# 3dhumangan/3DHumanGAN

Measured on NVIDIA H100. Metric: images_per_sec_G_fwd_512x512, higher is better.
Workload: dtype f32 (bf16x3 split on wgmma, fp32 accumulate)

## Files before the change

3dhumangan_b200/csrc/synth.cu:

```cuda
#include "common.cuh"
#include "wgmma.cuh"

namespace hg {

constexpr int kC = 256;
constexpr int kSynThreads = 384;
constexpr int kSynStages = 2;
constexpr int kASlots = 2;
constexpr int kXSlots = 5;
constexpr int kXs = 3;
constexpr int kSs = 2;
constexpr uint32_t kAChunk = 128 * 128;
constexpr uint32_t kBStage = 256 * 128;
constexpr uint32_t kXSlice = 32 * 128 * 4;

struct SpadeArgs {
  const float* x;
  long x_bstride;
  const float* mod;
  const float* scsh;
  const float* p_lr;
  long p_stride;
  const float* p_bias;
  const uint8_t* wgb;
  const float* bgb;
  const uint8_t* wimg;
  const float* bias;
  const float* skip;
  long skip_bstride;
  float* out;
  double* stats;
  const float* rgb_w;
  const float* rgb_b;
  const float* rgb_in;
  float* rgb_out;
  int B, HW, Hg, Wg, Rh, Rw;
  int nkc;
  int xC;
  const float* x2;
  float slope;
  int cout;
  int out_pm;
  int act;
  const float* ascale;
  const float* rk_v;
  int rk_n;
  const float* mod2;
};

struct SynSmem {
  uint8_t* a_hi;
  uint8_t* a_lo;
  uint8_t* b_st;
  float* x_st;
  int xs_n, ss_n;
  float* tab_g1;
  float* tab_g0;
  float* tab_bias;
  float* tab_rgbw;
  float* tab_bgb;
  float* tab_as;
  float* st_sum;
  float* st_sq;
  uint64_t* bars;
};

template <bool kPixel>
__device__ __forceinline__ SynSmem carve(uint8_t* raw) {
  constexpr int kA = kPixel ? 3 : kASlots, kX = kPixel ? 3 : kXSlots;
  uint8_t* s = reinterpret_cast<uint8_t*>((reinterpret_cast<uintptr_t>(raw) + 1023) & ~uintptr_t(1023));
  SynSmem m;
  m.a_hi = s;
  m.a_lo = s + kA * kAChunk;
  m.b_st = s + 2 * kA * kAChunk;
  m.x_st = reinterpret_cast<float*>(m.b_st + kSynStages * kBStage);
  m.xs_n = kPixel ? 2 : kXs;
  m.ss_n = kPixel ? 1 : kSs;
  float* f = m.x_st + kX * (kXSlice / 4);
  m.tab_g1 = f; f += kC;
  m.tab_g0 = f; f += kC;
  m.tab_bias = f; f += kC;
  m.tab_rgbw = f; f += 3 * kC;
  m.tab_bgb = f; f += 512;
  m.tab_as = f; f += kC;
  m.st_sum = f; f += kC;
  m.st_sq = f; f += kC;
  m.bars = reinterpret_cast<uint64_t*>(f);
  return m;
}
constexpr uint32_t kSynSmemBytes = 2 * kASlots * kAChunk + kSynStages * kBStage + kXSlots * kXSlice +
                                   (kC * 9 + 512) * 4 + 24 * 8 + 1024;
constexpr uint32_t kPixSmemBytes = 2 * 3 * kAChunk + kSynStages * kBStage + 3 * kXSlice + (kC * 9 + 512) * 4 + 24 * 8 + 1024;
static_assert(kSynSmemBytes <= 232448 && kPixSmemBytes <= 232448, "shared memory budget");

enum { B_FULL = 0 , B_EMPTY = 2 , X_FULL = 4 , X_EMPTY = 12  };

__device__ __forceinline__ void rows_barrier() { named_barrier(1, 256); }

__device__ __forceinline__ float lrelu02(float v) { return v > 0.f ? v : 0.2f * v; }

__device__ __forceinline__ float reduce_2pi(float t) {
  const float y = t * 0.15915494309189535f;
  const float k = (y + 12582912.f) - 12582912.f;
  float r = fmaf(-k, 6.2831854820251465f, t);
  return fmaf(-k, -1.7484555314695172e-07f, r);
}
__device__ __forceinline__ float sin_red(float t) { return __sinf(reduce_2pi(t)); }
__device__ __forceinline__ float cos_red(float t) { return __cosf(reduce_2pi(t)); }
__device__ __forceinline__ float2 reduce_2pi2(float2 t) {
  const float2 y = fmul2(t, make_float2(0.15915494309189535f, 0.15915494309189535f));
  const float2 k = fadd2(fadd2(y, make_float2(12582912.f, 12582912.f)), make_float2(-12582912.f, -12582912.f));
  const float2 r = ffma2(k, make_float2(-6.2831854820251465f, -6.2831854820251465f), t);
  return ffma2(k, make_float2(1.7484555314695172e-07f, 1.7484555314695172e-07f), r);
}
__device__ __forceinline__ float2 sin_red2(float2 t) { const float2 r = reduce_2pi2(t); return make_float2(__sinf(r.x), __sinf(r.y)); }
__device__ __forceinline__ float2 cos_red2(float2 t) { const float2 r = reduce_2pi2(t); return make_float2(__cosf(r.x), __cosf(r.y)); }

struct TileMap {
  int T, first, stride, count;
  __device__ __forceinline__ void get(int it, int& b, int& ti) const {
    const int tile = first + it * stride;
    b = tile / T;
    ti = tile - b * T;
  }
};

__device__ __forceinline__ void init_common(const SpadeArgs& a, const SynSmem& m) {
  for (int i = threadIdx.x; i < kC; i += blockDim.x) {
    m.tab_bias[i] = a.bias[i];
    m.st_sum[i] = 0.f;
    m.st_sq[i] = 0.f;
  }
  if (a.rgb_w)
    for (int i = threadIdx.x; i < 3 * kC; i += blockDim.x) m.tab_rgbw[i] = a.rgb_w[i];
  if (threadIdx.x == 0) {
    for (int i = 0; i < kSynStages; ++i) {
      mbar_init(m.bars + B_FULL + i, 1);
      mbar_init(m.bars + B_EMPTY + i, 2);
    }
    for (int i = 0; i < m.xs_n + m.ss_n; ++i) {
      mbar_init(m.bars + X_FULL + i, 1);
      mbar_init(m.bars + X_EMPTY + i, 8);
    }
    fence_mbar_init();
  }
  __syncthreads();
}

template <int kPasses>
__device__ __forceinline__ void weight_producer_loop(const SynSmem& m, const uint8_t* img, int nstages, int num_my_tiles) {
  uint32_t st = 0, ph = 0;
  for (int t = 0; t < num_my_tiles; ++t)
    for (int s = 0; s < nstages; ++s) {
      if (kPasses == 1 && (s & 1)) continue;
      mbar_wait_backoff(m.bars + B_EMPTY + st, ph ^ 1);
      mbar_arrive_expect_tx(m.bars + B_FULL + st, kBStage);
      bulk_g2s(m.b_st + st * kBStage, img + static_cast<size_t>(s) * kBStage, kBStage, m.bars + B_FULL + st);
      if (++st == kSynStages) { st = 0; ph ^= 1; }
    }
}

struct Pipe {
  uint32_t st = 0, ph = 0, prev = ~0u;
};
template <int N, int kPasses>
__device__ __forceinline__ void pipe_chunk(const SynSmem& m, Pipe& p, float (&d)[N / 2], uint32_t a_hi, uint32_t a_lo, bool accumulate,
                                           int t) {
#pragma unroll
  for (int part = 0; part < (kPasses == 3 ? 2 : 1); ++part) {
    mbar_wait(m.bars + B_FULL + p.st, p.ph);
    acc_fence(d);
    wgmma_fence();
    const uint32_t bt = smem_u32(m.b_st + p.st * kBStage);
    if (part == 0) {
      wg_k64<N>(d, a_hi, bt, accumulate);
      if (kPasses == 3) wg_k64<N>(d, a_lo, bt, true);
    } else {
      wg_k64<N>(d, a_hi, bt, true);
    }
    wgmma_commit();
    wgmma_wait<1>();
    acc_fence(d);
    if (p.prev != ~0u && t == 0) mbar_arrive(m.bars + B_EMPTY + p.prev);
    p.prev = p.st;
    if (++p.st == kSynStages) { p.st = 0; p.ph ^= 1; }
  }
}
template <int N>
__device__ __forceinline__ void pipe_drain(const SynSmem& m, Pipe& p, float (&d)[N / 2], int t) {
  wgmma_wait<0>();
  acc_fence(d);
  if (p.prev != ~0u && t == 0) mbar_arrive(m.bars + B_EMPTY + p.prev);
  p.prev = ~0u;
}

__device__ __forceinline__ void ring_emit(const SynSmem& m, uint32_t& g, int base, int slots, const float* src) {
  const uint32_t slot = base + g % slots;
  mbar_wait_backoff(m.bars + X_EMPTY + slot, ((g / slots) & 1) ^ 1);
  mbar_arrive_expect_tx(m.bars + X_FULL + slot, kXSlice);
  bulk_g2s(m.x_st + slot * (kXSlice / 4), src, kXSlice, m.bars + X_FULL + slot);
  ++g;
}
__device__ __forceinline__ void x_producer_loop(const SpadeArgs& a, const SynSmem& m, const TileMap& tm) {
  uint32_t g = 0;
  for (int it = 0; it < tm.count; ++it) {
    int b, ti;
    tm.get(it, b, ti);
    const int per_src = a.xC / 32;
    const float* base = a.x + static_cast<long>(b) * a.x_bstride + static_cast<long>(ti) * a.xC * 128;
    const float* base2 = a.x2 ? a.x2 + (static_cast<long>(b) * tm.T + ti) * a.xC * 128 : nullptr;
    for (int j = 0; j < 2 * a.nkc; ++j)
      ring_emit(m, g, 0, m.xs_n, (j < per_src ? base : base2 - per_src * 32 * 128) + j * 32 * 128);
  }
}
__device__ __forceinline__ void skip_producer_loop(const SpadeArgs& a, const SynSmem& m, const TileMap& tm) {
  if (!a.skip) return;
  uint32_t g = 0;
  for (int it = 0; it < tm.count; ++it) {
    int b, ti;
    tm.get(it, b, ti);
    const float* base = a.skip + static_cast<long>(b) * a.skip_bstride + static_cast<long>(ti) * a.cout * 128;
    for (int j = 0; j < a.cout / 32; ++j) ring_emit(m, g, m.xs_n, m.ss_n, base + j * 32 * 128);
  }
}

__device__ __forceinline__ uint32_t ring_take(const SynSmem& m, uint32_t g, int base, int slots) {
  const uint32_t slot = base + g % slots;
  mbar_wait_sleep(m.bars + X_FULL + slot, (g / slots) & 1);
  return slot;
}
__device__ __forceinline__ void ring_release(const SynSmem& m, uint32_t slot) {
  __syncwarp();
  if ((threadIdx.x & 31) == 0) mbar_arrive(m.bars + X_EMPTY + slot);
}

__device__ __forceinline__ void take_x_pair(const SynSmem& m, uint32_t& xg, int h, int row, float (&dst)[32]) {
#pragma unroll
  for (int hh = 0; hh < 2; ++hh, ++xg) {
    const uint32_t xslot = ring_take(m, xg, 0, m.xs_n);
    if (hh == h) {
      const uint32_t xs = smem_u32(m.x_st + xslot * (kXSlice / 4)) + row * 4;
#pragma unroll
      for (int j = 0; j < 32; ++j) dst[j] = lds_f32(xs + j * 512);
    }
    ring_release(m, xslot);
  }
}

__device__ __forceinline__ void column_sums(float* st, int c0, const float (&v)[4][2]) {
  const int lane = threadIdx.x & 31, r = lane >> 2;
  const bool b2 = r & 4, b1 = r & 2, b0 = r & 1;
  float w[4], u[2];
#pragma unroll
  for (int i = 0; i < 4; ++i) {
    const float lo = v[i >> 1][i & 1], hi = v[(i + 4) >> 1][i & 1];
    w[i] = (b2 ? hi : lo) + __shfl_xor_sync(0xffffffffu, b2 ? lo : hi, 16);
  }
#pragma unroll
  for (int i = 0; i < 2; ++i)
    u[i] = (b1 ? w[i + 2] : w[i]) + __shfl_xor_sync(0xffffffffu, b1 ? w[i] : w[i + 2], 8);
  const float x = (b0 ? u[1] : u[0]) + __shfl_xor_sync(0xffffffffu, b0 ? u[0] : u[1], 4);
  atomicAdd(st + c0 + 8 * (r >> 1) + 2 * (lane & 3) + (r & 1), x);
}

template <bool kSkip>
__device__ __forceinline__ void epilogue_fwd(const SpadeArgs& a, const SynSmem& m, const float (&d)[128], int b, int ti, int T,
                                             int g, int t, uint32_t& sg) {
  const int HW = a.HW, cout = a.cout;
  const bool kRgb = a.rgb_w != nullptr, kStats = a.stats != nullptr;
  int row[2];
  bool valid[2];
#pragma unroll
  for (int i = 0; i < 2; ++i) {
    row[i] = g * 64 + frag_row(t, i);
    valid[i] = ti * 128 + row[i] < HW;
  }
  float* const otile = a.out + (static_cast<long>(b) * T + ti) * cout * 128;
  float r[2][3] = {{0.f, 0.f, 0.f}, {0.f, 0.f, 0.f}};
#pragma unroll
  for (int cg = 0; cg < 8; ++cg) {
    if (cg * 32 >= cout) break;
    float sk[2][4][2];
    if (kSkip) {
      const uint32_t slot = ring_take(m, sg, m.xs_n, m.ss_n);
      const float* xs = m.x_st + slot * (kXSlice / 4);
#pragma unroll
      for (int i = 0; i < 2; ++i)
#pragma unroll
        for (int jj = 0; jj < 4; ++jj)
#pragma unroll
          for (int e = 0; e < 2; ++e) sk[i][jj][e] = xs[(frag_col(t, jj, e)) * 128 + row[i]];
      ring_release(m, slot);
      ++sg;
    }
    float s1[4][2], s2[4][2];
#pragma unroll
    for (int jj = 0; jj < 4; ++jj)
#pragma unroll
      for (int e = 0; e < 2; ++e) {
        const int j = cg * 4 + jj, c = frag_col(t, j, e);
        const float bc = m.tab_bias[c];
        s1[jj][e] = 0.f;
        s2[jj][e] = 0.f;
#pragma unroll
        for (int i = 0; i < 2; ++i) {
          float v = d[4 * j + 2 * i + e] + bc;
          if (kSkip) v += sk[i][jj][e];
          if (valid[i]) otile[c * 128 + row[i]] = v;
          else v = 0.f;
          if (kRgb) {
#pragma unroll
            for (int k = 0; k < 3; ++k) r[i][k] = fmaf(v, m.tab_rgbw[k * kC + c], r[i][k]);
          }
          s1[jj][e] += v;
          s2[jj][e] = fmaf(v, v, s2[jj][e]);
        }
      }
    if (kStats) {
      column_sums(m.st_sum, cg * 32, s1);
      column_sums(m.st_sq, cg * 32, s2);
    }
  }
  if (kRgb) {
#pragma unroll
    for (int i = 0; i < 2; ++i) {
#pragma unroll
      for (int k = 0; k < 3; ++k) {
        r[i][k] += __shfl_xor_sync(0xffffffffu, r[i][k], 1);
        r[i][k] += __shfl_xor_sync(0xffffffffu, r[i][k], 2);
      }
      if ((t & 3) == 0 && valid[i]) {
        const int pix = ti * 128 + row[i];
#pragma unroll
        for (int k = 0; k < 3; ++k) {
          const long idx = (static_cast<long>(b) * 3 + k) * HW + pix;
          float o = r[i][k] + a.rgb_b[k];
          if (a.rgb_in) o += a.rgb_in[idx];
          a.rgb_out[idx] = o;
        }
      }
    }
  }
}

__device__ __forceinline__ void epilogue_fwd_any(const SpadeArgs& a, const SynSmem& m, const float (&d)[128], int b, int ti, int T,
                                                 int g, int t, uint32_t& sg) {
  if (a.skip) epilogue_fwd<true>(a, m, d, b, ti, T, g, t, sg);
  else epilogue_fwd<false>(a, m, d, b, ti, T, g, t, sg);
}

__device__ __forceinline__ void flush_fwd_stats(const SpadeArgs& a, const SynSmem& m) {
  rows_barrier();
  if (a.stats)
    for (int c = threadIdx.x; c < kC; c += 256) {
      atomicAdd(a.stats + c, static_cast<double>(m.st_sum[c]));
      atomicAdd(a.stats + kC + c, static_cast<double>(m.st_sq[c]));
    }
}

template <bool kSine, bool kRk, bool kPm>
__device__ __forceinline__ void epilogue_bwd(const SpadeArgs& a, const SynSmem& m, const float (&d)[128], int b, int ti, int T, int g,
                                             int t, uint32_t& sg) {
  const int HW = a.HW, cout = a.cout, rk_n = a.rk_n;
  const float mslope = a.slope;
  int row[2];
  bool valid[2];
  float rv[2][3] = {{0.f, 0.f, 0.f}, {0.f, 0.f, 0.f}};
#pragma unroll
  for (int i = 0; i < 2; ++i) {
    row[i] = g * 64 + frag_row(t, i);
    valid[i] = ti * 128 + row[i] < HW;
    if (kRk && valid[i]) {
      const float* rp = a.rk_v + static_cast<long>(b) * rk_n * HW + ti * 128 + row[i];
      rv[i][0] = rp[0];
      if (rk_n > 1) rv[i][1] = rp[HW];
      if (rk_n > 2) rv[i][2] = rp[2 * static_cast<long>(HW)];
    }
  }
  float* const otile = a.out + (static_cast<long>(b) * T + ti) * cout * 128;
#pragma unroll
  for (int cg = 0; cg < 8; ++cg) {
    if (cg * 32 >= cout) break;
    float xv[2][4][2];
    {
      const uint32_t slot = ring_take(m, sg, m.xs_n, m.ss_n);
      const float* xs = m.x_st + slot * (kXSlice / 4);
#pragma unroll
      for (int i = 0; i < 2; ++i)
#pragma unroll
        for (int jj = 0; jj < 4; ++jj)
#pragma unroll
          for (int e = 0; e < 2; ++e)
            xv[i][jj][e] = valid[i] ? xs[frag_col(t, jj, e) * 128 + row[i]] : 0.f;
      ring_release(m, slot);
      ++sg;
    }
    float s1[4][2], s2[4][2];
#pragma unroll
    for (int jj = 0; jj < 4; ++jj)
#pragma unroll
      for (int e = 0; e < 2; ++e) {
        const int j = cg * 4 + jj, c = frag_col(t, j, e);
        const float t1 = m.tab_g1[c], t0 = m.tab_g0[c];
        s1[jj][e] = 0.f;
        s2[jj][e] = 0.f;
#pragma unroll
        for (int i = 0; i < 2; ++i) {
          const float x = xv[i][jj][e];
          const float pre = fmaf(x, t1, t0);
          float acc = d[4 * j + 2 * i + e];
          if (kRk)
            acc = fmaf(rv[i][2], m.tab_rgbw[2 * kC + c], fmaf(rv[i][1], m.tab_rgbw[kC + c], fmaf(rv[i][0], m.tab_rgbw[c], acc)));
          const float mask = kSine ? cos_red(pre) : (pre > 0.f ? 1.f : mslope);
          const float dd = acc * mask;
          if (valid[i]) {
            if (kPm) a.out[(static_cast<long>(b) * HW + ti * 128 + row[i]) * cout + c] = dd;
            else otile[c * 128 + row[i]] = dd;
          }
          s1[jj][e] += dd;
          s2[jj][e] = fmaf(dd, x, s2[jj][e]);
        }
      }
    column_sums(m.st_sum, cg * 32, s1);
    column_sums(m.st_sq, cg * 32, s2);
  }
}

__device__ __forceinline__ void epilogue_bwd_any(const SpadeArgs& a, const SynSmem& m, const float (&d)[128], int b, int ti, int T,
                                                 int g, int t, uint32_t& sg) {
  if (a.act == 1) {
    if (a.rk_v) epilogue_bwd<true, true, false>(a, m, d, b, ti, T, g, t, sg);
    else epilogue_bwd<true, false, false>(a, m, d, b, ti, T, g, t, sg);
  } else {
    if (a.out_pm) epilogue_bwd<false, false, true>(a, m, d, b, ti, T, g, t, sg);
    else epilogue_bwd<false, false, false>(a, m, d, b, ti, T, g, t, sg);
  }
}

__device__ __forceinline__ void flush_bwd_sums(const SpadeArgs& a, const SynSmem& m, int b) {
  for (int c = threadIdx.x; c < a.cout; c += 256) {
    atomicAdd(a.stats + (static_cast<long>(b) * 2 + 0) * a.cout + c, static_cast<double>(m.st_sum[c]));
    atomicAdd(a.stats + (static_cast<long>(b) * 2 + 1) * a.cout + c, static_cast<double>(m.st_sq[c]));
    m.st_sum[c] = 0.f;
    m.st_sq[c] = 0.f;
  }
}

template <int kPasses, bool kBwd>
__global__ void __launch_bounds__(kSynThreads, 1) spade_const_kernel(SpadeArgs a) {
  extern __shared__ uint8_t smem_raw[];
  const SynSmem m = carve<false>(smem_raw);
  const int warp = threadIdx.x >> 5, lane = threadIdx.x & 31;
  init_common(a, m);
  TileMap tm;
  tm.T = (a.HW + 127) / 128;
  tm.first = blockIdx.x;
  tm.stride = gridDim.x;
  tm.count = (a.B * tm.T - static_cast<int>(blockIdx.x) + static_cast<int>(gridDim.x) - 1) / static_cast<int>(gridDim.x);

  if (warp < 8) {
    regs_inc<kMmaRegs>();
    const int g = warp >> 2, t = threadIdx.x & 127;
    const int q = 2 * g + (warp & 1), h = (warp >> 1) & 1;
    const int row = q * 32 + lane;
    int cur_b = -1;
    uint32_t acnt = 0;
    uint32_t xg = 0, sg = 0;
    Pipe p;
    float d[128];
    for (int it = 0; it < tm.count; ++it) {
      int b, ti;
      tm.get(it, b, ti);
      if (b != cur_b) {
        rows_barrier();
        if (kBwd && cur_b >= 0) flush_bwd_sums(a, m, cur_b);
        for (int i = threadIdx.x; i < kC; i += 256) {
          if (kBwd) {
            if (a.ascale) {
              const long ld = a.x2 ? 2 * kC : kC;
              m.tab_as[i] = a.ascale[static_cast<long>(b) * ld + i];
              if (a.x2) m.tab_bgb[i] = a.ascale[static_cast<long>(b) * ld + kC + i];
            }
            if (i < a.cout) {
              m.tab_g1[i] = a.mod ? a.mod[(static_cast<long>(b) * 2 + 0) * a.cout + i] : 1.f;
              m.tab_g0[i] = a.mod ? a.mod[(static_cast<long>(b) * 2 + 1) * a.cout + i] : 0.f;
            }
          } else {
            m.tab_g1[i] = a.mod ? a.mod[(static_cast<long>(b) * 2 + 0) * kC + i] : 1.f;
            m.tab_g0[i] = a.mod ? a.mod[(static_cast<long>(b) * 2 + 1) * kC + i] : 0.f;
            if (a.mod2) {
              m.tab_bgb[i] = a.mod2[(static_cast<long>(b) * 2 + 0) * kC + i];
              m.tab_bgb[kC + i] = a.mod2[(static_cast<long>(b) * 2 + 1) * kC + i];
            }
          }
        }
        rows_barrier();
        cur_b = b;
      }
      const bool valid = ti * 128 + row < a.HW;
      uint32_t tg1a = smem_u32(kBwd ? m.tab_as : m.tab_g1), tg0a = smem_u32(m.tab_g0);
      uint32_t tg1b = smem_u32(m.tab_bgb), tg0b = smem_u32(m.tab_bgb + kC);
      opaque(tg1a);
      opaque(tg0a);
      opaque(tg1b);
      opaque(tg0b);
      const float slope = a.slope;
      const bool sine = a.act == 1, scaled = kBwd && a.ascale != nullptr;
      const bool two_tables = kBwd ? (scaled && a.x2 != nullptr) : a.mod2 != nullptr;
#pragma unroll 1
      for (int kc = 0; kc < a.nkc; ++kc, ++acnt) {
        const int c0 = (kc * 64 + h * 32) & (kC - 1);
        const bool second = two_tables && kc * 64 >= kC;
        const uint32_t tg1 = second ? tg1b : tg1a, tg0 = second ? tg0b : tg0a;
        float cur[32];
        take_x_pair(m, xg, h, row, cur);
        const uint32_t slot = acnt & 1;
#pragma unroll
        for (int gi = 0; gi < 4; ++gi) {
          float y[8], t1[8], t0[8];
          if (!kBwd || scaled) lds8(tg1 + (c0 + gi * 8) * 4, t1);
          if (!kBwd) lds8(tg0 + (c0 + gi * 8) * 4, t0);
          if (kBwd) {
#pragma unroll
            for (int j = 0; j < 8; ++j) y[j] = scaled ? cur[gi * 8 + j] * t1[j] : cur[gi * 8 + j];
          } else if (sine) {
#pragma unroll
            for (int j = 0; j < 8; j += 2) {
              const float2 sv = sin_red2(ffma2(make_float2(cur[gi * 8 + j], cur[gi * 8 + j + 1]), make_float2(t1[j], t1[j + 1]),
                                               make_float2(t0[j], t0[j + 1])));
              y[j] = sv.x;
              y[j + 1] = sv.y;
            }
          } else {
            affine_lrelu8(cur + gi * 8, t1, t0, slope, y);
          }
          if (!valid) {
#pragma unroll
            for (int j = 0; j < 8; ++j) y[j] = 0.f;
          }
          store_a8<kPasses == 3>(m.a_hi + slot * kAChunk, m.a_lo + slot * kAChunk, row, h * 32 + gi * 8, y);
        }
        fence_proxy_async_smem();
        named_barrier(2 + g, 128);
        pipe_chunk<256, kPasses>(m, p, d, smem_u32(m.a_hi + slot * kAChunk) + g * 64 * 128,
                                 smem_u32(m.a_lo + slot * kAChunk) + g * 64 * 128, kc > 0, t);
      }
      pipe_drain<256>(m, p, d, t);
      if (kBwd) epilogue_bwd_any(a, m, d, b, ti, tm.T, g, t, sg);
      else epilogue_fwd_any(a, m, d, b, ti, tm.T, g, t, sg);
    }
    if (kBwd) {
      rows_barrier();
      if (cur_b >= 0) flush_bwd_sums(a, m, cur_b);
    } else {
      flush_fwd_stats(a, m);
    }
  } else {
    regs_dec<kProducerRegs>();
    if (lane == 0) {
      if (warp == 8) weight_producer_loop<kPasses>(m, a.wimg, 2 * a.nkc, tm.count);
      else if (warp == 9) x_producer_loop(a, m, tm);
      else if (warp == 10) skip_producer_loop(a, m, tm);
    }
  }
}

__device__ __forceinline__ void bilin(int dst, int in_size, float scale, int& i0, int& i1, float& l0, float& l1) {
  float src = scale * (static_cast<float>(dst) + 0.5f) - 0.5f;
  src = src < 0.f ? 0.f : src;
  i0 = static_cast<int>(src);
  i1 = i0 + (i0 < in_size - 1 ? 1 : 0);
  l1 = src - static_cast<float>(i0);
  l0 = 1.f - l1;
}

template <int kPasses>
__device__ __forceinline__ void pixel_weight_producer_loop(const SpadeArgs& a, const SynSmem& m, int num_my_tiles) {
  uint32_t st = 0, ph = 0;
  auto emit = [&](const uint8_t* src, uint32_t bytes) {
    mbar_wait_backoff(m.bars + B_EMPTY + st, ph ^ 1);
    mbar_arrive_expect_tx(m.bars + B_FULL + st, bytes);
    bulk_g2s(m.b_st + st * kBStage, src, bytes, m.bars + B_FULL + st);
    if (++st == kSynStages) { st = 0; ph ^= 1; }
  };
  for (int t = 0; t < num_my_tiles; ++t)
    for (int kc = 0; kc < 4; ++kc) {
      for (int k = 0; k < 2; ++k)
        for (int part = 0; part < (kPasses == 3 ? 2 : 1); ++part)
          emit(a.wgb + static_cast<size_t>(((kc >> 1) * 2 + k) * 2 + part) * kBStage + (kc & 1) * (kBStage / 2), kBStage / 2);
      for (int part = 0; part < (kPasses == 3 ? 2 : 1); ++part) emit(a.wimg + static_cast<size_t>(kc * 2 + part) * kBStage, kBStage);
    }
}

template <int kPasses>
__global__ void __launch_bounds__(kSynThreads, 1) spade_pixel_kernel(SpadeArgs a) {
  extern __shared__ uint8_t smem_raw[];
  const SynSmem m = carve<true>(smem_raw);
  const int warp = threadIdx.x >> 5, lane = threadIdx.x & 31;
  for (int i = threadIdx.x; i < kC; i += blockDim.x) {
    m.tab_g1[i] = a.scsh[i];
    m.tab_g0[i] = a.scsh[kC + i];
  }
  for (int i = threadIdx.x; i < 512; i += blockDim.x) m.tab_bgb[i] = a.bgb[i];
  init_common(a, m);
  TileMap tm;
  tm.T = (a.HW + 127) / 128;
  tm.first = blockIdx.x;
  tm.stride = gridDim.x;
  tm.count = (a.B * tm.T - static_cast<int>(blockIdx.x) + static_cast<int>(gridDim.x) - 1) / static_cast<int>(gridDim.x);
  const float sy = static_cast<float>(a.Rh) / static_cast<float>(a.Hg);
  const float sx = static_cast<float>(a.Rw) / static_cast<float>(a.Wg);

  if (warp < 8) {
    regs_inc<kMmaRegs>();
    const int g = warp >> 2, t = threadIdx.x & 127;
    const int q = 2 * g + (warp & 1), h = (warp >> 1) & 1;
    const int row = q * 32 + lane;
    uint8_t* const y_hi = m.a_hi + 2 * kAChunk;
    uint8_t* const y_lo = m.a_lo + 2 * kAChunk;
    uint32_t xg = 0, sg = 0;
    Pipe p;
    float d[128], e[64];
    for (int it = 0; it < tm.count; ++it) {
      int b, ti;
      tm.get(it, b, ti);
      const int pix = ti * 128 + row;
      const bool valid = pix < a.HW;
      {
        const int py = valid ? pix / a.Wg : 0, px = valid ? pix % a.Wg : 0;
        int y0, y1, x0, x1;
        float ly0, ly1, lx0, lx1;
        bilin(py, a.Rh, sy, y0, y1, ly0, ly1);
        bilin(px, a.Rw, sx, x0, x1, lx0, lx1);
        const float* base = a.p_lr + static_cast<long>(b) * a.Rh * a.Rw * a.p_stride;
        const float4* n00 = reinterpret_cast<const float4*>(base + (static_cast<long>(y0) * a.Rw + x0) * a.p_stride);
        const float4* n01 = reinterpret_cast<const float4*>(base + (static_cast<long>(y0) * a.Rw + x1) * a.p_stride);
        const float4* n10 = reinterpret_cast<const float4*>(base + (static_cast<long>(y1) * a.Rw + x0) * a.p_stride);
        const float4* n11 = reinterpret_cast<const float4*>(base + (static_cast<long>(y1) * a.Rw + x1) * a.p_stride);
        const float4* pb = a.p_bias ? reinterpret_cast<const float4*>(a.p_bias + static_cast<long>(b) * 128) : nullptr;
        const float2 lx0p = make_float2(lx0, lx0), lx1p = make_float2(lx1, lx1), ly0p = make_float2(ly0, ly0), ly1p = make_float2(ly1, ly1);
#pragma unroll 2
        for (int gi = 0; gi < 8; ++gi) {
          float y[8];
#pragma unroll
          for (int u = 0; u < 2; ++u) {
            const int f4 = h * 16 + gi * 2 + u;
            const float4 v00 = __ldg(n00 + f4), v01 = __ldg(n01 + f4), v10 = __ldg(n10 + f4), v11 = __ldg(n11 + f4);
            auto lerp2 = [&](float2 a, float2 b, float2 c, float2 d) {
              const float2 top = ffma2(b, lx1p, fmul2(a, lx0p));
              const float2 bot = ffma2(d, lx1p, fmul2(c, lx0p));
              return ffma2(top, ly0p, fmul2(bot, ly1p));
            };
            float2 lo2 = lerp2(make_float2(v00.x, v00.y), make_float2(v01.x, v01.y), make_float2(v10.x, v10.y), make_float2(v11.x, v11.y));
            float2 hi2 = lerp2(make_float2(v00.z, v00.w), make_float2(v01.z, v01.w), make_float2(v10.z, v10.w), make_float2(v11.z, v11.w));
            if (pb) {
              const float4 c4 = __ldg(pb + f4);
              lo2 = fadd2(lo2, make_float2(c4.x, c4.y));
              hi2 = fadd2(hi2, make_float2(c4.z, c4.w));
            }
            y[u * 4 + 0] = lo2.x; y[u * 4 + 1] = lo2.y; y[u * 4 + 2] = hi2.x; y[u * 4 + 3] = hi2.y;
          }
#pragma unroll
          for (int j = 0; j < 8; ++j) y[j] = valid ? fmaxf(y[j], 0.f) : 0.f;
          store_a8<kPasses == 3>(m.a_hi + h * kAChunk, m.a_lo + h * kAChunk, row, gi * 8, y);
        }
        fence_proxy_async_smem();
        named_barrier(2 + g, 128);
      }
      int frow[2];
      bool fvalid[2];
#pragma unroll
      for (int i = 0; i < 2; ++i) {
        frow[i] = g * 64 + frag_row(t, i);
        fvalid[i] = ti * 128 + frow[i] < a.HW;
      }
#pragma unroll 1
      for (int kc = 0; kc < 4; ++kc) {
        for (int k = 0; k < 2; ++k)
          pipe_chunk<128, kPasses>(m, p, e, smem_u32(m.a_hi + k * kAChunk) + g * 64 * 128, smem_u32(m.a_lo + k * kAChunk) + g * 64 * 128,
                                   k > 0, t);
        pipe_drain<128>(m, p, e, t);
        const uint32_t s0 = ring_take(m, xg, 0, m.xs_n), s1 = ring_take(m, xg + 1, 0, m.xs_n);
        xg += 2;
        const float* xs0 = m.x_st + s0 * (kXSlice / 4);
        const float* xs1 = m.x_st + s1 * (kXSlice / 4);
        const int col = (kc >> 1) * 256 + (kc & 1) * 128;
#pragma unroll
        for (int j = 0; j < 8; ++j) {
          const int c = frag_col(t, j, 0), ch = kc * 64 + c;
          const float* xs = j < 4 ? xs0 : xs1;
#pragma unroll
          for (int i = 0; i < 2; ++i) {
            float y2[2];
#pragma unroll
            for (int u = 0; u < 2; ++u) {
              const float gam = e[4 * j + 2 * i + u] + m.tab_bgb[col + c + u];
              const float bet = e[4 * (j + 8) + 2 * i + u] + m.tab_bgb[col + 64 + c + u];
              const float xn = fmaf(xs[((c + u) & 31) * 128 + frow[i]], m.tab_g1[ch + u], m.tab_g0[ch + u]);
              const float v = fmaf(xn, gam, bet);
              y2[u] = fvalid[i] ? fmaxf(v, 0.2f * v) : 0.f;
            }
            uint32_t hb, lb;
            split_bf16x2(y2[0], y2[1], hb, lb);
            const uint32_t off = sw128_offset(frow[i], c);
            asm volatile("st.shared.b32 [%0], %1;" ::"r"(smem_u32(y_hi) + off), "r"(hb));
            if (kPasses == 3) asm volatile("st.shared.b32 [%0], %1;" ::"r"(smem_u32(y_lo) + off), "r"(lb));
          }
        }
        ring_release(m, s0);
        ring_release(m, s1);
        fence_proxy_async_smem();
        named_barrier(2 + g, 128);
        pipe_chunk<256, kPasses>(m, p, d, smem_u32(y_hi) + g * 64 * 128, smem_u32(y_lo) + g * 64 * 128, kc > 0, t);
      }
      pipe_drain<256>(m, p, d, t);
      epilogue_fwd_any(a, m, d, b, ti, tm.T, g, t, sg);
    }
    flush_fwd_stats(a, m);
  } else {
    regs_dec<kProducerRegs>();
    if (lane == 0) {
      if (warp == 8) pixel_weight_producer_loop<kPasses>(a, m, tm.count);
      else if (warp == 9) x_producer_loop(a, m, tm);
      else if (warp == 10) skip_producer_loop(a, m, tm);
    }
  }
}

__global__ void bn_finalize_kernel(const double* __restrict__ stats, double count_in, const double* __restrict__ count_ptr,
                                   const float* __restrict__ weight,
                                   const float* __restrict__ bias, float* running_mean, float* running_var,
                                   int training, float eps, float momentum, const float* __restrict__ gb, int B,
                                   float* __restrict__ scsh, float* __restrict__ mod) {
  const int c = threadIdx.x;
  float mean, var;
  const double count = count_ptr ? count_ptr[0] : count_in;
  if (training) {
    const double mu = stats[c] / count;
    double v = stats[kC + c] / count - mu * mu;
    v = v < 0 ? 0 : v;
    mean = static_cast<float>(mu);
    var = static_cast<float>(v);
    if (running_mean) {
      const double unb = count > 1 ? v * count / (count - 1) : v;
      running_mean[c] = (1.f - momentum) * running_mean[c] + momentum * mean;
      running_var[c] = (1.f - momentum) * running_var[c] + momentum * static_cast<float>(unb);
    }
  } else {
    mean = running_mean[c];
    var = running_var[c];
  }
  const float sc = weight[c] * rsqrtf(var + eps);
  const float sh = bias[c] - mean * sc;
  if (scsh) {
    scsh[c] = sc;
    scsh[kC + c] = sh;
  }
  if (mod && gb) {
    for (int b = 0; b < B; ++b) {
      const float G = gb[(static_cast<long>(b) * 2 + 0) * kC + c];
      const float Bt = gb[(static_cast<long>(b) * 2 + 1) * kC + c];
      mod[(static_cast<long>(b) * 2 + 0) * kC + c] = sc * G;
      mod[(static_cast<long>(b) * 2 + 1) * kC + c] = fmaf(sh, G, Bt);
    }
  }
}

__global__ void synth_input_kernel(const float* __restrict__ w, const float* __restrict__ bias,
                                   const float* __restrict__ ic, const float* __restrict__ jc, int Hg, int Wg,
                                   float* __restrict__ x0, double* __restrict__ stats, double batch_mult) {
  const int c = blockIdx.y;
  const int HW = Hg * Wg;
  const float w0 = w[c * 2 + 0], w1 = w[c * 2 + 1], bb = bias[c];
  float s1 = 0.f, s2 = 0.f;
  for (int p = blockIdx.x * blockDim.x + threadIdx.x; p < HW; p += gridDim.x * blockDim.x) {
    const float v = sinf(fmaf(w1, jc[p % Wg], fmaf(w0, ic[p / Wg], bb)));
    x0[(static_cast<long>(p >> 7) * kC + c) * 128 + (p & 127)] = v;
    s1 += v;
    s2 += v * v;
  }
  __shared__ float r1[8], r2[8];
  for (int o = 16; o > 0; o >>= 1) {
    s1 += __shfl_xor_sync(0xffffffffu, s1, o);
    s2 += __shfl_xor_sync(0xffffffffu, s2, o);
  }
  if ((threadIdx.x & 31) == 0) { r1[threadIdx.x >> 5] = s1; r2[threadIdx.x >> 5] = s2; }
  __syncthreads();
  if (threadIdx.x == 0 && stats) {
    float t1 = 0.f, t2 = 0.f;
    for (int i = 0; i < static_cast<int>(blockDim.x >> 5); ++i) { t1 += r1[i]; t2 += r2[i]; }
    atomicAdd(stats + c, static_cast<double>(t1) * batch_mult);
    atomicAdd(stats + kC + c, static_cast<double>(t2) * batch_mult);
  }
}

}

extern "C" {

int hg_spade_conv(const float* x, long x_bstride, const float* mod, const float* scsh, const float* p_lr,
                  long p_stride, const float* p_bias, const void* wgb, const float* bgb, const void* wimg, const float* bias, const float* skip,
                  float* out, double* stats, const float* rgb_w, const float* rgb_b, const float* rgb_in,
                  float* rgb_out, int B, int C, int Hg, int Wg, int Rh, int Rw, int passes, void* stream) {
  HG_REQUIRE(C == hg::kC, "hg_spade_conv: only %d channels are supported (got %d)", hg::kC, C);
  HG_REQUIRE(x && wimg && bias && out, "hg_spade_conv: null pointer");
  HG_REQUIRE((mod != nullptr) != (p_lr != nullptr), "hg_spade_conv: give exactly one of mod (const style) / p_lr (pixel style)");
  HG_REQUIRE(passes == 1 || passes == 3, "hg_spade_conv: passes must be 1 or 3");
  HG_REQUIRE(B > 0 && Hg > 0 && Wg > 0, "hg_spade_conv: bad shape");
  HG_REQUIRE(!rgb_w || (rgb_b && rgb_out), "hg_spade_conv: rgb_b / rgb_out missing");
  if (p_lr) {
    HG_REQUIRE(scsh && wgb && bgb && Rh > 0 && Rw > 0, "hg_spade_conv: pixel-style arguments missing");
    HG_REQUIRE((reinterpret_cast<uintptr_t>(p_lr) & 15) == 0 && p_stride >= 128 && (p_stride & 3) == 0,
               "hg_spade_conv: p_lr must be 16-byte aligned with a row stride >= 128 that is a multiple of 4");
    HG_REQUIRE(!p_bias || (reinterpret_cast<uintptr_t>(p_bias) & 15) == 0, "hg_spade_conv: p_bias must be 16-byte aligned");
  }
  hg::SpadeArgs a{x, x_bstride, mod, scsh, p_lr, p_stride, p_bias, static_cast<const uint8_t*>(wgb), bgb,
                  static_cast<const uint8_t*>(wimg), bias, skip,
                  static_cast<long>((Hg * Wg + 127) / 128) * hg::kC * 128, out, stats, rgb_w, rgb_b, rgb_in, rgb_out,
                  B, Hg * Wg, Hg, Wg, Rh, Rw};
  a.nkc = 4; a.xC = hg::kC; a.x2 = nullptr; a.slope = 0.2f; a.cout = hg::kC; a.out_pm = 0;
  const int tiles = B * ((Hg * Wg + 127) / 128);
  const int grid = tiles < hg::num_sms() ? tiles : hg::num_sms();
  auto st = static_cast<cudaStream_t>(stream);
#define HG_LAUNCH(KERNEL, SMEM)                                                                                   \
  do {                                                                                                            \
    cudaError_t e = cudaFuncSetAttribute(KERNEL, cudaFuncAttributeMaxDynamicSharedMemorySize, SMEM);               \
    if (e != cudaSuccess) { hg::set_error("hg_spade_conv: smem opt-in failed: %s", cudaGetErrorString(e)); return 2; } \
    KERNEL<<<grid, hg::kSynThreads, SMEM, st>>>(a);                                                               \
  } while (0)
  if (mod) {
    if (passes == 3) HG_LAUNCH((hg::spade_const_kernel<3, false>), hg::kSynSmemBytes); else HG_LAUNCH((hg::spade_const_kernel<1, false>), hg::kSynSmemBytes);
  } else {
    if (passes == 3) HG_LAUNCH(hg::spade_pixel_kernel<3>, hg::kPixSmemBytes); else HG_LAUNCH(hg::spade_pixel_kernel<1>, hg::kPixSmemBytes);
  }
#undef HG_LAUNCH
  return hg::check_launch("hg_spade_conv");
}

static int launch_blocked_gemm(const hg::SpadeArgs& a, int passes, bool bwd, cudaStream_t st, const char* who) {
  const int tiles = a.B * ((a.HW + 127) / 128);
  const int grid = tiles < hg::num_sms() ? tiles : hg::num_sms();
  cudaError_t e;
#define HG_LAUNCH_G(KERNEL)                                                                             \
  do {                                                                                                  \
    e = cudaFuncSetAttribute(KERNEL, cudaFuncAttributeMaxDynamicSharedMemorySize, hg::kSynSmemBytes);   \
    if (e == cudaSuccess) KERNEL<<<grid, hg::kSynThreads, hg::kSynSmemBytes, st>>>(a);                   \
  } while (0)
  if (bwd) {
    if (passes == 3) HG_LAUNCH_G((hg::spade_const_kernel<3, true>)); else HG_LAUNCH_G((hg::spade_const_kernel<1, true>));
  } else {
    if (passes == 3) HG_LAUNCH_G((hg::spade_const_kernel<3, false>)); else HG_LAUNCH_G((hg::spade_const_kernel<1, false>));
  }
#undef HG_LAUNCH_G
  if (e != cudaSuccess) { hg::set_error("%s: smem opt-in failed: %s", who, cudaGetErrorString(e)); return 2; }
  return hg::check_launch(who);
}

int hg_spade_bwd_dgrad(const float* dout, const float* x, long x_bstride, const float* mod, const void* wimg_t, float* dpre,
                       double* sums, int B, int C, int Hg, int Wg, int passes, void* stream) {
  HG_REQUIRE(C == hg::kC, "hg_spade_bwd_dgrad: only %d channels are supported (got %d)", hg::kC, C);
  HG_REQUIRE(dout && x && mod && wimg_t && dpre && sums, "hg_spade_bwd_dgrad: null pointer");
  HG_REQUIRE(passes == 1 || passes == 3, "hg_spade_bwd_dgrad: passes must be 1 or 3");
  HG_REQUIRE(B > 0 && Hg > 0 && Wg > 0, "hg_spade_bwd_dgrad: bad shape");
  const long T = (Hg * Wg + 127) / 128;
  hg::SpadeArgs a{};
  a.x = dout;
  a.x_bstride = T * hg::kC * 128;
  a.mod = mod;
  a.wimg = static_cast<const uint8_t*>(wimg_t);
  a.bias = mod;
  a.skip = x;
  a.skip_bstride = x_bstride;
  a.out = dpre;
  a.stats = sums;
  a.B = B; a.HW = Hg * Wg; a.Hg = Hg; a.Wg = Wg;
  a.nkc = 4; a.xC = hg::kC; a.slope = 0.2f; a.cout = hg::kC;
  return launch_blocked_gemm(a, passes, true, static_cast<cudaStream_t>(stream), "hg_spade_bwd_dgrad");
}

int hg_conv1x1_blocked(const float* x, int Cin, const void* wimg, const float* bias, float* out, int B, int Hg, int Wg,
                       int passes, void* stream) {
  HG_REQUIRE(x && wimg && bias && out, "hg_conv1x1_blocked: null pointer");
  HG_REQUIRE(Cin == 64 || Cin == 128 || Cin == 256, "hg_conv1x1_blocked: Cin must be 64, 128 or 256 (got %d)", Cin);
  HG_REQUIRE(passes == 1 || passes == 3, "hg_conv1x1_blocked: passes must be 1 or 3");
  HG_REQUIRE(B > 0 && Hg > 0 && Wg > 0, "hg_conv1x1_blocked: bad shape");
  const long T = (Hg * Wg + 127) / 128;
  hg::SpadeArgs a{};
  a.x = x;
  a.x_bstride = T * Cin * 128;
  a.wimg = static_cast<const uint8_t*>(wimg);
  a.bias = bias;
  a.skip_bstride = T * hg::kC * 128;
  a.out = out;
  a.B = B; a.HW = Hg * Wg; a.Hg = Hg; a.Wg = Wg;
  a.nkc = Cin / 64; a.xC = Cin; a.slope = 1.f; a.cout = hg::kC;
  return launch_blocked_gemm(a, passes, false, static_cast<cudaStream_t>(stream), "hg_conv1x1_blocked");
}

int hg_act_conv1x1_blocked(const float* x, const float* x2, const float* mod, int act, const void* wimg, const float* bias,
                           float* out, int B, int Hg, int Wg, int passes, void* stream) {
  HG_REQUIRE(x && mod && wimg && bias && out, "hg_act_conv1x1_blocked: null pointer");
  HG_REQUIRE(act == 0 || act == 1, "hg_act_conv1x1_blocked: act must be 0 (LeakyReLU 0.2) or 1 (sine)");
  HG_REQUIRE(passes == 1 || passes == 3, "hg_act_conv1x1_blocked: passes must be 1 or 3");
  HG_REQUIRE(B > 0 && Hg > 0 && Wg > 0, "hg_act_conv1x1_blocked: bad shape");
  const long T = (Hg * Wg + 127) / 128;
  hg::SpadeArgs a{};
  a.x = x;
  a.x_bstride = T * hg::kC * 128;
  a.x2 = x2;
  a.mod = mod;
  a.wimg = static_cast<const uint8_t*>(wimg);
  a.bias = bias;
  a.skip_bstride = T * hg::kC * 128;
  a.out = out;
  a.B = B; a.HW = Hg * Wg; a.Hg = Hg; a.Wg = Wg;
  a.nkc = x2 ? 8 : 4; a.xC = hg::kC; a.slope = 0.2f; a.cout = hg::kC; a.act = act;
  return launch_blocked_gemm(a, passes, false, static_cast<cudaStream_t>(stream), "hg_act_conv1x1_blocked");
}

int hg_blocked_conv_wide(const float* x, const float* x2, const float* mod, const float* mod2, int act, float slope,
                         const void* wimg, const float* bias, const float* skip, float* out, double* stats,
                         const float* rgb_w, const float* rgb_b, const float* rgb_in, float* rgb_out, int B, int Hg, int Wg,
                         int passes, void* stream) {
  HG_REQUIRE(x && wimg && bias && out, "hg_blocked_conv_wide: null pointer");
  HG_REQUIRE(act == 0 || act == 1, "hg_blocked_conv_wide: act must be 0 (LeakyReLU(slope)) or 1 (sine)");
  HG_REQUIRE(!mod2 || (mod && x2), "hg_blocked_conv_wide: mod2 needs mod and a second source");
  HG_REQUIRE(!rgb_w || (rgb_b && rgb_out), "hg_blocked_conv_wide: rgb_b / rgb_out missing");
  HG_REQUIRE(passes == 1 || passes == 3, "hg_blocked_conv_wide: passes must be 1 or 3");
  HG_REQUIRE(B > 0 && Hg > 0 && Wg > 0, "hg_blocked_conv_wide: bad shape");
  const long T = (Hg * Wg + 127) / 128;
  hg::SpadeArgs a{};
  a.x = x;
  a.x_bstride = T * hg::kC * 128;
  a.x2 = x2;
  a.mod = mod;
  a.mod2 = mod2;
  a.wimg = static_cast<const uint8_t*>(wimg);
  a.bias = bias;
  a.skip = skip;
  a.skip_bstride = T * hg::kC * 128;
  a.out = out;
  a.stats = stats;
  a.rgb_w = rgb_w; a.rgb_b = rgb_b; a.rgb_in = rgb_in; a.rgb_out = rgb_out;
  a.B = B; a.HW = Hg * Wg; a.Hg = Hg; a.Wg = Wg;
  a.nkc = x2 ? 8 : 4; a.xC = hg::kC; a.slope = slope; a.cout = hg::kC; a.act = act;
  return launch_blocked_gemm(a, passes, false, static_cast<cudaStream_t>(stream), "hg_blocked_conv_wide");
}

int hg_conv1x1_blocked_bwd(const float* g, const float* g2, const float* aux, const float* mod, const void* wimg_t,
                           float* out, double* sums, int Cout, float slope, int pixel_major, int act, const float* ascale,
                           const float* rk_w, const float* rk_v, int rk_n, int B, int Hg, int Wg, int passes,
                           void* stream) {
  HG_REQUIRE(act == 0 || act == 1, "hg_conv1x1_blocked_bwd: act must be 0 (LeakyReLU/ReLU mask) or 1 (cosine)");
  HG_REQUIRE(!rk_v || (rk_w && rk_n >= 1 && rk_n <= 3 && Cout == 256), "hg_conv1x1_blocked_bwd: bad rank-k term");
  HG_REQUIRE(g && aux && wimg_t && out && sums, "hg_conv1x1_blocked_bwd: null pointer");
  HG_REQUIRE(Cout == 128 || Cout == 256, "hg_conv1x1_blocked_bwd: Cout must be 128 or 256 (got %d)", Cout);
  HG_REQUIRE(!pixel_major || Cout == 128, "hg_conv1x1_blocked_bwd: the pixel-major output is built for Cout == 128");
  HG_REQUIRE(!(act == 1 && pixel_major) && !(act == 0 && rk_v),
             "hg_conv1x1_blocked_bwd: compiled epilogues are sine [+ rank-k term] / LeakyReLU [+ pixel-major output]");
  HG_REQUIRE(passes == 1 || passes == 3, "hg_conv1x1_blocked_bwd: passes must be 1 or 3");
  HG_REQUIRE(B > 0 && Hg > 0 && Wg > 0, "hg_conv1x1_blocked_bwd: bad shape");
  const long T = (Hg * Wg + 127) / 128;
  hg::SpadeArgs a{};
  a.x = g;
  a.x_bstride = T * hg::kC * 128;
  a.x2 = g2;
  a.mod = mod;
  a.wimg = static_cast<const uint8_t*>(wimg_t);
  a.bias = static_cast<const float*>(wimg_t);
  a.skip = aux;
  a.skip_bstride = T * Cout * 128;
  a.out = out;
  a.stats = sums;
  a.B = B; a.HW = Hg * Wg; a.Hg = Hg; a.Wg = Wg;
  a.nkc = g2 ? 8 : 4; a.xC = hg::kC; a.slope = slope; a.cout = Cout; a.out_pm = pixel_major;
  a.act = act; a.ascale = ascale; a.rgb_w = rk_v ? rk_w : nullptr; a.rk_v = rk_v; a.rk_n = rk_n;
  return launch_blocked_gemm(a, passes, true, static_cast<cudaStream_t>(stream), "hg_conv1x1_blocked_bwd");
}

int hg_bn_finalize(const double* stats, double count, const double* count_dev, const float* weight, const float* bias, float* running_mean,
                   float* running_var, int training, float eps, float momentum, const float* gb, int B, int C,
                   float* scsh, float* mod, void* stream) {
  HG_REQUIRE(C == hg::kC, "hg_bn_finalize: only %d channels are supported (got %d)", hg::kC, C);
  HG_REQUIRE(weight && bias && (scsh || mod), "hg_bn_finalize: null pointer");
  HG_REQUIRE(training ? (stats != nullptr && (count > 0 || count_dev)) : (running_mean && running_var),
             "hg_bn_finalize: statistics missing");
  hg::bn_finalize_kernel<<<1, hg::kC, 0, static_cast<cudaStream_t>(stream)>>>(
      stats, count, count_dev, weight, bias, running_mean, running_var, training, eps, momentum, gb, B, scsh, mod);
  return hg::check_launch("hg_bn_finalize");
}

int hg_synth_input(const float* w, const float* bias, const float* ic, const float* jc, int C, int Hg, int Wg,
                   float* x0, double* stats, int batch, void* stream) {
  HG_REQUIRE(C == hg::kC, "hg_synth_input: only %d channels are supported (got %d)", hg::kC, C);
  HG_REQUIRE(w && bias && ic && jc && x0, "hg_synth_input: null pointer");
  const int HW = Hg * Wg;
  int bx = (HW + 255) / 256;
  if (bx > 32) bx = 32;
  dim3 grid(bx, C);
  hg::synth_input_kernel<<<grid, 256, 0, static_cast<cudaStream_t>(stream)>>>(w, bias, ic, jc, Hg, Wg, x0, stats,
                                                                              static_cast<double>(batch));
  return hg::check_launch("hg_synth_input");
}

}
```

Baseline: 99.14.

## Split pixel-kernel weight ring into four half-stage units with finer-grained release

The pixel SPADE kernel's weight ring is re-tiled into four half-size units, each with its own full and empty mbarrier. The producer now always issues half-stage bulk copies, and the consumer waits and releases per unit through a new PixPipe. Freed slots go back to the producer sooner, so the next weight copy can overlap the current wgmma more deeply. The A1 build is moved into a helper with full unrolling, and the accumulators are explicitly zeroed, which costs extra instructions and register pressure.

```diff
diff --git a/3dhumangan_b200/csrc/synth.cu b/3dhumangan_b200/csrc/synth.cu
--- a/3dhumangan_b200/csrc/synth.cu
+++ b/3dhumangan_b200/csrc/synth.cu
@@ -93,7 +93,11 @@
 constexpr uint32_t kPixSmemBytes = 2 * 3 * kAChunk + kSynStages * kBStage + 3 * kXSlice + (kC * 9 + 512) * 4 + 24 * 8 + 1024;
 static_assert(kSynSmemBytes <= 232448 && kPixSmemBytes <= 232448, "shared memory budget");
 
-enum { B_FULL = 0 , B_EMPTY = 2 , X_FULL = 4 , X_EMPTY = 12  };
+constexpr int kPixUnits = 4;
+constexpr uint32_t kPixUnit = kBStage / 2;
+static_assert(kPixUnits * kPixUnit == kSynStages * kBStage, "the pixel-style units tile the weight ring");
+
+enum { B_FULL = 0 , B_EMPTY = 4 , X_FULL = 8 , X_EMPTY = 13  };
 
 __device__ __forceinline__ void rows_barrier() { named_barrier(1, 256); }
 
@@ -125,7 +129,7 @@
   }
 };
 
-__device__ __forceinline__ void init_common(const SpadeArgs& a, const SynSmem& m) {
+__device__ __forceinline__ void init_common(const SpadeArgs& a, const SynSmem& m, int weight_slots) {
   for (int i = threadIdx.x; i < kC; i += blockDim.x) {
     m.tab_bias[i] = a.bias[i];
     m.st_sum[i] = 0.f;
@@ -134,7 +138,7 @@
   if (a.rgb_w)
     for (int i = threadIdx.x; i < 3 * kC; i += blockDim.x) m.tab_rgbw[i] = a.rgb_w[i];
   if (threadIdx.x == 0) {
-    for (int i = 0; i < kSynStages; ++i) {
+    for (int i = 0; i < weight_slots; ++i) {
       mbar_init(m.bars + B_FULL + i, 1);
       mbar_init(m.bars + B_EMPTY + i, 2);
     }
@@ -451,7 +455,7 @@
   extern __shared__ uint8_t smem_raw[];
   const SynSmem m = carve<false>(smem_raw);
   const int warp = threadIdx.x >> 5, lane = threadIdx.x & 31;
-  init_common(a, m);
+  init_common(a, m, kSynStages);
   TileMap tm;
   tm.T = (a.HW + 127) / 128;
   tm.first = blockIdx.x;
@@ -576,20 +580,112 @@
 
 template <int kPasses>
 __device__ __forceinline__ void pixel_weight_producer_loop(const SpadeArgs& a, const SynSmem& m, int num_my_tiles) {
-  uint32_t st = 0, ph = 0;
-  auto emit = [&](const uint8_t* src, uint32_t bytes) {
-    mbar_wait_backoff(m.bars + B_EMPTY + st, ph ^ 1);
-    mbar_arrive_expect_tx(m.bars + B_FULL + st, bytes);
-    bulk_g2s(m.b_st + st * kBStage, src, bytes, m.bars + B_FULL + st);
-    if (++st == kSynStages) { st = 0; ph ^= 1; }
+  uint32_t n = 0;
+  auto emit = [&](const uint8_t* src) {
+    const uint32_t u = n % kPixUnits;
+    mbar_wait_backoff(m.bars + B_EMPTY + u, ((n / kPixUnits) & 1) ^ 1);
+    mbar_arrive_expect_tx(m.bars + B_FULL + u, kPixUnit);
+    bulk_g2s(m.b_st + u * kPixUnit, src, kPixUnit, m.bars + B_FULL + u);
+    ++n;
   };
   for (int t = 0; t < num_my_tiles; ++t)
     for (int kc = 0; kc < 4; ++kc) {
       for (int k = 0; k < 2; ++k)
         for (int part = 0; part < (kPasses == 3 ? 2 : 1); ++part)
-          emit(a.wgb + static_cast<size_t>(((kc >> 1) * 2 + k) * 2 + part) * kBStage + (kc & 1) * (kBStage / 2), kBStage / 2);
-      for (int part = 0; part < (kPasses == 3 ? 2 : 1); ++part) emit(a.wimg + static_cast<size_t>(kc * 2 + part) * kBStage, kBStage);
-    }
+          emit(a.wgb + static_cast<size_t>(((kc >> 1) * 2 + k) * 2 + part) * kBStage + (kc & 1) * kPixUnit);
+      for (int part = 0; part < (kPasses == 3 ? 2 : 1); ++part) {
+        const uint8_t* src = a.wimg + static_cast<size_t>(kc * 2 + part) * kBStage;
+        emit(src);
+        emit(src + kPixUnit);
+      }
+    }
+}
+
+struct PixPipe {
+  uint32_t n = 0;
+  uint32_t prev = 0;
+  uint32_t prev_units = 0;
+};
+__device__ __forceinline__ void pix_release(const SynSmem& m, PixPipe& p, int t) {
+  if (t == 0)
+    for (uint32_t j = 0; j < p.prev_units; ++j) mbar_arrive(m.bars + B_EMPTY + (p.prev + j) % kPixUnits);
+  p.prev_units = 0;
+}
+template <int N, int kPasses>
+__device__ __forceinline__ void pix_part(const SynSmem& m, PixPipe& p, float (&d)[N / 2], uint32_t a_hi, uint32_t a_lo, int part,
+                                         bool accumulate, int t) {
+  constexpr uint32_t kUnits = N == 256 ? 2 : 1;
+  const uint32_t u = p.n % kPixUnits;
+#pragma unroll
+  for (uint32_t j = 0; j < kUnits; ++j) mbar_wait(m.bars + B_FULL + u + j, ((p.n + j) / kPixUnits) & 1);
+  acc_fence(d);
+  wgmma_fence();
+  const uint32_t bt = smem_u32(m.b_st + u * kPixUnit);
+  if (part == 0) {
+    wg_k64<N>(d, a_hi, bt, accumulate);
+    if (kPasses == 3) wg_k64<N>(d, a_lo, bt, true);
+  } else {
+    wg_k64<N>(d, a_hi, bt, true);
+  }
+  wgmma_commit();
+  wgmma_wait<1>();
+  acc_fence(d);
+  pix_release(m, p, t);
+  p.prev = u;
+  p.prev_units = kUnits;
+  p.n += kUnits;
+}
+template <int N>
+__device__ __forceinline__ void pix_drain(const SynSmem& m, PixPipe& p, float (&d)[N / 2], int t) {
+  wgmma_wait<0>();
+  acc_fence(d);
+  pix_release(m, p, t);
+}
+
+template <int kPasses>
+__device__ __forceinline__ void build_a1(const SpadeArgs& a, const SynSmem& m, int b, int ti, int row, int h, int g, float sy,
+                                         float sx) {
+  const int pix = ti * 128 + row;
+  const bool valid = pix < a.HW;
+  const int py = valid ? pix / a.Wg : 0, px = valid ? pix % a.Wg : 0;
+  int y0, y1, x0, x1;
+  float ly0, ly1, lx0, lx1;
+  bilin(py, a.Rh, sy, y0, y1, ly0, ly1);
+  bilin(px, a.Rw, sx, x0, x1, lx0, lx1);
+  const float* base = a.p_lr + static_cast<long>(b) * a.Rh * a.Rw * a.p_stride;
+  const float4* n00 = reinterpret_cast<const float4*>(base + (static_cast<long>(y0) * a.Rw + x0) * a.p_stride);
+  const float4* n01 = reinterpret_cast<const float4*>(base + (static_cast<long>(y0) * a.Rw + x1) * a.p_stride);
+  const float4* n10 = reinterpret_cast<const float4*>(base + (static_cast<long>(y1) * a.Rw + x0) * a.p_stride);
+  const float4* n11 = reinterpret_cast<const float4*>(base + (static_cast<long>(y1) * a.Rw + x1) * a.p_stride);
+  const float4* pb = a.p_bias ? reinterpret_cast<const float4*>(a.p_bias + static_cast<long>(b) * 128) : nullptr;
+  const float2 lx0p = make_float2(lx0, lx0), lx1p = make_float2(lx1, lx1), ly0p = make_float2(ly0, ly0), ly1p = make_float2(ly1, ly1);
+#pragma unroll
+  for (int gi = 0; gi < 8; ++gi) {
+    float y[8];
+#pragma unroll
+    for (int u = 0; u < 2; ++u) {
+      const int f4 = h * 16 + gi * 2 + u;
+      const float4 v00 = __ldg(n00 + f4), v01 = __ldg(n01 + f4), v10 = __ldg(n10 + f4), v11 = __ldg(n11 + f4);
+      auto lerp2 = [&](float2 a, float2 b, float2 c, float2 d) {
+        const float2 top = ffma2(b, lx1p, fmul2(a, lx0p));
+        const float2 bot = ffma2(d, lx1p, fmul2(c, lx0p));
+        return ffma2(top, ly0p, fmul2(bot, ly1p));
+      };
+      float2 lo2 = lerp2(make_float2(v00.x, v00.y), make_float2(v01.x, v01.y), make_float2(v10.x, v10.y), make_float2(v11.x, v11.y));
+      float2 hi2 = lerp2(make_float2(v00.z, v00.w), make_float2(v01.z, v01.w), make_float2(v10.z, v10.w), make_float2(v11.z, v11.w));
+      if (pb) {
+        const float4 c4 = __ldg(pb + f4);
+        lo2 = fadd2(lo2, make_float2(c4.x, c4.y));
+        hi2 = fadd2(hi2, make_float2(c4.z, c4.w));
+      }
+      y[u * 4 + 0] = lo2.x; y[u * 4 + 1] = lo2.y; y[u * 4 + 2] = hi2.x; y[u * 4 + 3] = hi2.y;
+    }
+#pragma unroll
+    for (int j = 0; j < 8; ++j) y[j] = valid ? fmaxf(y[j], 0.f) : 0.f;
+    store_a8<kPasses == 3>(m.a_hi + h * kAChunk, m.a_lo + h * kAChunk, row, gi * 8, y);
+  }
+  fence_proxy_async_smem();
+  named_barrier(2 + g, 128);
 }
 
 template <int kPasses>
@@ -602,7 +698,7 @@
     m.tab_g0[i] = a.scsh[kC + i];
   }
   for (int i = threadIdx.x; i < 512; i += blockDim.x) m.tab_bgb[i] = a.bgb[i];
-  init_common(a, m);
+  init_common(a, m, kPixUnits);
   TileMap tm;
   tm.T = (a.HW + 127) / 128;
   tm.first = blockIdx.x;
@@ -618,55 +714,18 @@
     const int row = q * 32 + lane;
     uint8_t* const y_hi = m.a_hi + 2 * kAChunk;
     uint8_t* const y_lo = m.a_lo + 2 * kAChunk;
+    constexpr int kParts = kPasses == 3 ? 2 : 1;
     uint32_t xg = 0, sg = 0;
-    Pipe p;
+    PixPipe p;
     float d[128], e[64];
     for (int it = 0; it < tm.count; ++it) {
       int b, ti;
       tm.get(it, b, ti);
-      const int pix = ti * 128 + row;
-      const bool valid = pix < a.HW;
-      {
-        const int py = valid ? pix / a.Wg : 0, px = valid ? pix % a.Wg : 0;
-        int y0, y1, x0, x1;
-        float ly0, ly1, lx0, lx1;
-        bilin(py, a.Rh, sy, y0, y1, ly0, ly1);
-        bilin(px, a.Rw, sx, x0, x1, lx0, lx1);
-        const float* base = a.p_lr + static_cast<long>(b) * a.Rh * a.Rw * a.p_stride;
-        const float4* n00 = reinterpret_cast<const float4*>(base + (static_cast<long>(y0) * a.Rw + x0) * a.p_stride);
-        const float4* n01 = reinterpret_cast<const float4*>(base + (static_cast<long>(y0) * a.Rw + x1) * a.p_stride);
-        const float4* n10 = reinterpret_cast<const float4*>(base + (static_cast<long>(y1) * a.Rw + x0) * a.p_stride);
-        const float4* n11 = reinterpret_cast<const float4*>(base + (static_cast<long>(y1) * a.Rw + x1) * a.p_stride);
-        const float4* pb = a.p_bias ? reinterpret_cast<const float4*>(a.p_bias + static_cast<long>(b) * 128) : nullptr;
-        const float2 lx0p = make_float2(lx0, lx0), lx1p = make_float2(lx1, lx1), ly0p = make_float2(ly0, ly0), ly1p = make_float2(ly1, ly1);
-#pragma unroll 2
-        for (int gi = 0; gi < 8; ++gi) {
-          float y[8];
-#pragma unroll
-          for (int u = 0; u < 2; ++u) {
-            const int f4 = h * 16 + gi * 2 + u;
-            const float4 v00 = __ldg(n00 + f4), v01 = __ldg(n01 + f4), v10 = __ldg(n10 + f4), v11 = __ldg(n11 + f4);
-            auto lerp2 = [&](float2 a, float2 b, float2 c, float2 d) {
-              const float2 top = ffma2(b, lx1p, fmul2(a, lx0p));
-              const float2 bot = ffma2(d, lx1p, fmul2(c, lx0p));
-              return ffma2(top, ly0p, fmul2(bot, ly1p));
-            };
-            float2 lo2 = lerp2(make_float2(v00.x, v00.y), make_float2(v01.x, v01.y), make_float2(v10.x, v10.y), make_float2(v11.x, v11.y));
-            float2 hi2 = lerp2(make_float2(v00.z, v00.w), make_float2(v01.z, v01.w), make_float2(v10.z, v10.w), make_float2(v11.z, v11.w));
-            if (pb) {
-              const float4 c4 = __ldg(pb + f4);
-              lo2 = fadd2(lo2, make_float2(c4.x, c4.y));
-              hi2 = fadd2(hi2, make_float2(c4.z, c4.w));
-            }
-            y[u * 4 + 0] = lo2.x; y[u * 4 + 1] = lo2.y; y[u * 4 + 2] = hi2.x; y[u * 4 + 3] = hi2.y;
-          }
-#pragma unroll
-          for (int j = 0; j < 8; ++j) y[j] = valid ? fmaxf(y[j], 0.f) : 0.f;
-          store_a8<kPasses == 3>(m.a_hi + h * kAChunk, m.a_lo + h * kAChunk, row, gi * 8, y);
-        }
-        fence_proxy_async_smem();
-        named_barrier(2 + g, 128);
-      }
+      build_a1<kPasses>(a, m, b, ti, row, h, g, sy, sx);
+#pragma unroll
+      for (int i = 0; i < 128; ++i) d[i] = 0.f;
+#pragma unroll
+      for (int i = 0; i < 64; ++i) e[i] = 0.f;
       int frow[2];
       bool fvalid[2];
 #pragma unroll
@@ -676,10 +735,13 @@
       }
 #pragma unroll 1
       for (int kc = 0; kc < 4; ++kc) {
-        for (int k = 0; k < 2; ++k)
-          pipe_chunk<128, kPasses>(m, p, e, smem_u32(m.a_hi + k * kAChunk) + g * 64 * 128, smem_u32(m.a_lo + k * kAChunk) + g * 64 * 128,
-                                   k > 0, t);
-        pipe_drain<128>(m, p, e, t);
+#pragma unroll
+        for (int s = 0; s < 2 * kParts; ++s) {
+          const int k = s / kParts;
+          pix_part<128, kPasses>(m, p, e, smem_u32(m.a_hi + k * kAChunk) + g * 64 * 128, smem_u32(m.a_lo + k * kAChunk) + g * 64 * 128,
+                                 s % kParts, s > 0, t);
+        }
+        pix_drain<128>(m, p, e, t);
         const uint32_t s0 = ring_take(m, xg, 0, m.xs_n), s1 = ring_take(m, xg + 1, 0, m.xs_n);
         xg += 2;
         const float* xs0 = m.x_st + s0 * (kXSlice / 4);
@@ -711,9 +773,11 @@
         ring_release(m, s1);
         fence_proxy_async_smem();
         named_barrier(2 + g, 128);
-        pipe_chunk<256, kPasses>(m, p, d, smem_u32(y_hi) + g * 64 * 128, smem_u32(y_lo) + g * 64 * 128, kc > 0, t);
+#pragma unroll
+        for (int part = 0; part < kParts; ++part)
+          pix_part<256, kPasses>(m, p, d, smem_u32(y_hi) + g * 64 * 128, smem_u32(y_lo) + g * 64 * 128, part, kc > 0, t);
       }
-      pipe_drain<256>(m, p, d, t);
+      pix_drain<256>(m, p, d, t);
       epilogue_fwd_any(a, m, d, b, ti, tm.T, g, t, sg);
     }
     flush_fwd_stats(a, m);
```

Result: faster. 102.3, median of 6 (+3.2%).
